# hherlyng/knp-emi-cgx

Hardware: AMD Instinct MI355X
Metric: MDoF/s per implicit timestep (assembly+GMRES) (higher is better)
Workload: dtype f64

## Files before the change

include/knpemi_hip.h:

```cpp
#ifndef KNPEMI_HIP_H
#define KNPEMI_HIP_H

#include <stdint.h>

#ifdef __cplusplus
extern "C" {
#endif

#define KNP_MAX_IONS 3
#define KNP_MAX_AUX 8
#define KNP_DIAG_MAX_CONSTS 64
#define KNP_MAX_PROG_REGS 48
#define KNP_STATE_MAX_INSTR 768
#define KNP_STATE_MAX_CONSTS 128
#define KNP_MAX_AMG_LEVELS 16
#define KNP_FUNCTIONAL_MAX_Q 125

#define KNP_OK 0
#define KNP_E_ARG (-1)
#define KNP_E_HIP (-2)
#define KNP_E_STATE (-3)
#define KNP_E_ALLOC (-4)
#define KNP_E_MESH (-5)

// ... 222 lines not shown
                         double rhs_scale, double* b);
int knp_emi_pc_setup(knp_ctx* ctx, int32_t kind);
int knp_emi_pc_apply(knp_ctx* ctx, const double* r, double* z);
int knp_emi_cg_solve(knp_ctx* ctx, const double* b, double* x, double rtol, double atol, int32_t max_it, int32_t norm_type,
                     int32_t* its, double* rnorm, int32_t* reason);
int knp_emi_update(knp_ctx* ctx, const double* x, double* phi_i, double* phi_e, double* phi_m);

int knp_timer_mark(knp_ctx* ctx, int32_t join_assembly);
int knp_timer_read(knp_ctx* ctx, int32_t capacity, double* seconds , int32_t* n_intervals);
int knp_timer_pending(const knp_ctx* ctx);
int knp_profile_enable(knp_ctx* ctx, int32_t class_mask);
int knp_profile_get(knp_ctx* ctx, int32_t cls, double* ms, int64_t* launches);
int knp_profile_reset(knp_ctx* ctx);
enum { KNP_ST_BNORM = 0 , KNP_ST_ALLREDUCE = 1 ,
       KNP_ST_HALO = 2 , KNP_ST_READBACK = 3 ,
       KNP_ST_FUSED = 4 ,
       KNP_ST_NORM_FALLBACK = 5 ,
       KNP_ST_BLOCKED = 6 ,
       KNP_ST_FUSED_LEVELS = 7 ,
       KNP_ST_FUSED_DOTS = 8 ,
       KNP_ST_SPMV_DOTS = 9 ,
       KNP_ST_FUSED_TAILS = 10 ,
       KNP_ST_KNOD_SKIPS = 11 ,
       KNP_ST_COUNT = 12 };
int knp_get_stats(const knp_ctx* ctx, double* out );
int knp_get_traffic_model(const knp_ctx* ctx, double* out );
enum { KNP_LI_ASM_VARIANT = 0 ,
       KNP_LI_ASM_STAGE = 1 ,
       KNP_LI_ASM_DMAX = 2 ,
       KNP_LI_ASM_GROUP = 3, KNP_LI_SPMV_GROUP = 4, KNP_LI_PC_GROUP = 5 ,
       KNP_LI_MAX_NODE_CELLS = 6 ,
       KNP_LI_MAX_NODE_PAIRS = 7 ,
       KNP_LI_SPMV_UNROLL = 8 ,
       KNP_LI_SPMV_MK = 9 ,
       KNP_LI_COUNT = 10 };
int knp_get_launch_info(const knp_ctx* ctx, int32_t* out , int n);
enum { KNP_AI_A_LANES = 0, KNP_AI_P_LANES = 1, KNP_AI_R_LANES = 2, KNP_AI_S_LANES = 3, KNP_AI_RT_LANES = 4, KNP_AI_U_LANES = 5,
       KNP_AI_BA_LANES = 6, KNP_AI_BR_LANES = 7, KNP_AI_BS_LANES = 8, KNP_AI_BRT_LANES = 9, KNP_AI_BU_LANES = 10,
       KNP_AI_P_N_ACT = 11, KNP_AI_S_N_ACT = 12 ,
       KNP_AI_LFUSED = 13 ,
       KNP_AI_N = 14, KNP_AI_N_COARSE = 15, KNP_AI_FP32 = 16 ,
       KNP_AI_H_FUSED = 17, KNP_AI_H_BLOCKED = 18, KNP_AI_H_CFUSED = 19, KNP_AI_H_L0_FUSED = 20 ,
       KNP_AI_H_NC = 21 ,
       KNP_AI_H_CINV_F32 = 22 ,
       KNP_AI_COUNT = 23 };
int knp_amg_get_level_info(const knp_ctx* ctx, int32_t hier, int32_t level, int32_t* out , int n);

// ... 5 lines not shown
```

knp-emi-cgx_amd/cgx_hip/backend.py:

```python
from __future__ import annotations

import ctypes as C
import os

import numpy as np
import torch

from . import _lib
from ._lib import Fields, FieldsOut, KnpError, MeshDesc
from .parallel import HaloPlan, all_reduce_sum_, guarded


class _CAI:

    def __init__(self, ptr, n):
        self.__cuda_array_interface__ = {"shape": (int(n),), "typestr": "<f8", "data": (int(ptr), False),
                                         "version": 2, "strides": None}


def _f64(a):
    return a.ctypes.data_as(_lib.f64p)


def _i32(a):
# ... 665 lines not shown
    def timer_pending(self):
        return int(self.lib.knp_timer_pending(self.ctx))

    def timer_read(self):
        n = self.timer_pending()
        if n < 2:
            if n:
                out = (C.c_double * 1)()
                k = C.c_int32()
                self.check(self.lib.knp_timer_read(self.ctx, 1, out, C.byref(k)))
            return np.zeros(0)
        out = (C.c_double * n)()
        k = C.c_int32()
        self.check(self.lib.knp_timer_read(self.ctx, n, out, C.byref(k)))
        return np.array(out[:k.value], dtype=np.float64)

    def profile_enable(self, mask=0x1f):
        self.check(self.lib.knp_profile_enable(self.ctx, int(mask)))

    def profile_reset(self):
        self.check(self.lib.knp_profile_reset(self.ctx))

    def stats(self):
        out = (C.c_double * 12)()
        self.check(self.lib.knp_get_stats(self.ctx, out))
        return {"bnorm": out[0], "allreduces": int(out[1]), "halos": int(out[2]), "readbacks": int(out[3]), "fused": int(out[4]),
                "norm_fallbacks": int(out[5]), "blocked": int(out[6]), "fused_levels": int(out[7]),
                "fused_dots": int(out[8]), "spmv_dots": int(out[9]), "fused_tails": int(out[10]), "knod_skips": int(out[11])}

    def nodal_conc(self):
        out = np.empty((self.n_nodes, 4), dtype=np.float64)
        self.check(self.lib.knp_get_nodal_conc(self.ctx, _f64(out)))
        return out

    def traffic_model(self):
        out = (C.c_double * 5)()
        self.check(self.lib.knp_get_traffic_model(self.ctx, out))
        return {"spmv": out[0], "pc": out[1], "assembly_matrix": out[2], "assembly_rhs": out[3], "vector": out[4]}

    def launch_info(self):
        names = ["asm_variant", "asm_stage", "asm_dmax", "asm_group", "spmv_group", "pc_group", "max_node_cells", "max_node_pairs",
                 "spmv_unroll", "spmv_mk"]
        out = (C.c_int32 * len(names))()
        self.check(self.lib.knp_get_launch_info(self.ctx, out, len(names)))
        return dict(zip(names, (int(v) for v in out)))

    AMG_LEVEL_INFO = ["A_lanes", "P_lanes", "R_lanes", "S_lanes", "Rt_lanes", "U_lanes", "bA_lanes", "bR_lanes", "bS_lanes", "bRt_lanes",
                      "bU_lanes", "P_n_act", "S_n_act", "lfused", "n", "n_coarse", "fp32", "fused", "blocked", "cfused", "l0_fused", "nc", "cinv_f32"]

    def amg_level_info(self, hier, level):
        out = (C.c_int32 * len(self.AMG_LEVEL_INFO))()
# ... 13 lines not shown
```

knp-emi-cgx_amd/csrc/knp_internal.hpp:

```cpp
#pragma once
#include <hip/hip_runtime.h>

#include <cstdint>
#include <string>
#include <vector>

#include "knpemi_hip.h"

#define KNP_NPROF 5

struct KnpHostGraph {
    int dim = 0, nv1 = 0;
    int n_v = 0, n_v_owned = 0, n_c = 0, n_c_owned = 0, n_g = 0, n_q = 0;
    int n_nodes = 0, n_nodes_owned = 0;
    std::vector<int32_t> node_i, node_e;
    std::vector<int32_t> node_vertex;
    std::vector<uint8_t> node_side;
    std::vector<int32_t> pair_ptr;
    std::vector<int32_t> pair_col;
    std::vector<int32_t> pair_row;
    std::vector<double> pair_M, pair_K;
    std::vector<int32_t> contrib_ptr;
    std::vector<int32_t> contrib_cell;
    std::vector<double> contrib_k;
// ... 330 lines not shown
    void* comm_user = nullptr;
    KnpP2P* p2p = nullptr;
    int p2p_fine = -1;
    int p2p_red = -1;
    bool hook_allreduce() const { return allreduce && p2p_red < 0; }
    int comm_rc = 0;
    int n_int = 0, n_bnd = 0;
    int32_t *d_nodes_int = nullptr, *d_nodes_bnd = nullptr;
    hipStream_t stream3 = nullptr;
    hipEvent_t ev_x = nullptr, ev_halo = nullptr;
    hipStream_t stream2 = nullptr;
    hipEvent_t ev_fork = nullptr, ev_join = nullptr;
    KnpSidePrep prep;
    bool side_ws = false;
    double *d_t2_s = nullptr, *d_w2_s = nullptr, *d_wb = nullptr, *d_partial_s = nullptr;
    hipStream_t stream_asm = nullptr;
    hipEvent_t ev_fork_asm = nullptr, ev_asm = nullptr;
    bool asm_pending = false;
    double last_bnorm = 0.0;
    int64_t n_allreduce = 0, n_halo = 0, n_readback = 0;
    int64_t n_fused_dots = 0;
    int64_t n_spmv_dots = 0;
    int fused_tail = 1;
    int update_early = 1;
    bool tail_ok = false;
    bool have_tail_target = false;
    knp_fields_out tail_target = {};
    const double* tail_x = nullptr;
    bool fields_current = false, knod_current = false, fields_promise = false;
    bool knod_skipped = false;
    int64_t n_fused_tail = 0;
    int64_t n_knod_skip = 0;
    std::vector<hipEvent_t> tm_events;
    size_t tm_used = 0;
    KnpDiagMap diag_cells, diag_facets;
    KnpDiagMap diag_flux;
    double2* d_flux_rec = nullptr;
    KnpDiagMap diag_phim;
    int32_t* diag_code = nullptr;
    int diag_n_instr = 0, diag_n_regs = 0, diag_n_consts = 0;
    double diag_consts[KNP_DIAG_MAX_CONSTS] = {};
    bool diag_prog = false;
    KnpEmi emi;
    KnpStates states;
    std::vector<KnpSamplePlan> sample_plans;
    std::vector<KnpFunctional> functionals;
// ... 11 lines not shown
```

knp-emi-cgx_amd/csrc/knp_kernels.hip:

```cpp
#include <hip/hip_runtime.h>
#include <hip/hip_ext.h>

#include <algorithm>
#include <cmath>
#include <cstdio>
#include <cstdlib>
#include <cstring>
#include <new>

#include "knp_dispatch.hpp"
#include "knp_internal.hpp"

#define HIPCHK(call)                                                                       \
    do {                                                                                   \
        hipError_t e_ = (call);                                                            \
        if (e_ != hipSuccess) {                                                            \
            ctx->err = std::string(#call) + ": " + hipGetErrorString(e_);                  \
            return KNP_E_HIP;                                                              \
        }                                                                                  \
    } while (0)
#define KCHK(expr)                         \
    do {                                   \
        int rc_ = (expr);                  \
        if (rc_ != KNP_OK) return rc_;     \
// ... 1565 lines not shown
    static const double scale_r = getenv("KNP_LANE_SCALE_R") ? atof(getenv("KNP_LANE_SCALE_R")) : 1.0;
    avg_nnz_per_row *= scale * (role == 1 ? scale_p : role == 2 ? scale_r : 1.0);
    if (avg_nnz_per_row <= 8.0) return 2;
    if (avg_nnz_per_row <= 16.0) return 4;
    if (avg_nnz_per_row <= 32.0) return 8;
    if (avg_nnz_per_row <= 80.0) return 16;
    if (avg_nnz_per_row <= 192.0) return 32;
    return 64;
}

struct GmLayout {
    int m;
    __host__ __device__ int H(int i, int j) const { return i + j * (m + 1); }
    __host__ __device__ int cs() const { return (m + 1) * m; }
    __host__ __device__ int sn() const { return cs() + m; }
    __host__ __device__ int g() const { return sn() + m; }
    __host__ __device__ int y() const { return g() + m + 1; }
    __host__ __device__ int st() const { return y() + m; }
    __host__ __device__ int size() const { return st() + 8; }
};
static constexpr double GM_CANCEL = 1e-8;

__device__ __forceinline__ void givens_body(GmLayout L, int j, int has_ns, double inv_cnt, const double* __restrict__ red, int explicit_slot,
                                            double* __restrict__ gm, double* mirror, volatile int64_t* seq, int64_t seq_val) {
    double* st = gm + L.st();
    double nrm2;
    bool cancel = false;
    if (explicit_slot < 0) {
        const double ww = red[j + 1 + has_ns];
        double s = 0.0;
        for (int i = 0; i <= j; ++i) s += red[i] * red[i];
        if (has_ns) s += red[j + 1] * red[j + 1] * inv_cnt;
        nrm2 = ww - s;
        cancel = !(nrm2 > GM_CANCEL * ww) && ww > 0.0;
    } else {
        nrm2 = red[explicit_slot];
    }
    double flag = 0.0, res = 0.0;
    if (cancel) {
        flag = 1.0;
        nrm2 = 1.0;
    } else {
        double* h = gm + L.H(0, j);
        for (int i = 0; i <= j; ++i) h[i] = red[i];
        h[j + 1] = sqrt(fmax(nrm2, 0.0));
        double* cs = gm + L.cs();
        double* sn = gm + L.sn();
        double* g = gm + L.g();
        for (int i = 0; i < j; ++i) {
            const double t = cs[i] * h[i] + sn[i] * h[i + 1];
            h[i + 1] = -sn[i] * h[i] + cs[i] * h[i + 1];
            h[i] = t;
        }
        const double den = hypot(h[j], h[j + 1]);
        if (!(den > 0.0) || !isfinite(den) || !(nrm2 == nrm2)) {
            flag = 2.0;
            nrm2 = 1.0;
        } else {
            cs[j] = h[j] / den;
            sn[j] = h[j + 1] / den;
            h[j] = den;
            h[j + 1] = 0.0;
            g[j + 1] = -sn[j] * g[j];
            g[j] = cs[j] * g[j];
            res = fabs(g[j + 1]);
            if (!(nrm2 > 0.0)) nrm2 = 1.0;
        }
    }
    st[0] = nrm2; st[1] = flag; st[2] = res;
    if (mirror) { mirror[0] = res; mirror[1] = flag; }
    if (seq) {
        __threadfence_system();
        *seq = seq_val;
    }
}
__global__ void k_givens(GmLayout L, int j, int has_ns, double inv_cnt, const double* __restrict__ red, int explicit_slot,
                         double* __restrict__ gm, double* mirror, volatile int64_t* seq, int64_t seq_val) {
    if (threadIdx.x != 0) return;
    givens_body(L, j, has_ns, inv_cnt, red, explicit_slot, gm, mirror, seq, seq_val);
}

__device__ __forceinline__ void proj_norm_body(double s, double ww, double* __restrict__ red, int slot_out, double inv_count, double cancel, double* mirror,
                                               volatile int64_t* seq, int64_t seq_val) {
    const double nrm2 = ww - s * s * inv_count;
    const bool bad = !(nrm2 > cancel * ww) && ww > 0.0;
    red[slot_out] = bad ? ww : nrm2;
    red[slot_out + 1] = bad ? 1.0 : 0.0;
    if (mirror) { mirror[slot_out] = red[slot_out]; mirror[slot_out + 1] = red[slot_out + 1]; }
    if (seq) {
        __threadfence_system();
        *seq = seq_val;
    }
}
__device__ __forceinline__ void reduce_partial_rows(int nb, int nred, const double* __restrict__ partial, int stride, double* s_red) {
    const int wave = threadIdx.x >> 6, lane = threadIdx.x & 63;
    for (int row = wave; row < nred; row += NT / 64) {
        double a = 0.0;
        for (int c = 0; c < nb; c += 1024) {
            double v[16];
#pragma unroll
            for (int k = 0; k < 16; ++k) {
                const int b = c + lane + 64 * k;
                v[k] = b < nb ? partial[(size_t)row * stride + b] : 0.0;
            }
#pragma unroll
            for (int k = 0; k < 16; ++k) a += v[k];
        }
        a = wave_sum(a);
        if (lane == 0) s_red[row] = a;
    }
    __syncthreads();
}
__global__ void __launch_bounds__(NT)
k_reduce_fin(int mode, int nb, int nred, const double* __restrict__ partial, double* __restrict__ red, int slot0, GmLayout L, int j, int has_ns,
             double inv_cnt, double* __restrict__ gm, int slot_out, double cancel, double* mirror, volatile int64_t* seq, int64_t seq_val,
             int stride = RED_BLOCKS) {
    __shared__ double s_red[RED_SLOTS];
    reduce_partial_rows(nb, nred, partial, stride, s_red);
    if (threadIdx.x < nred) red[slot0 + threadIdx.x] = s_red[threadIdx.x];
// ... 65 lines not shown
            __threadfence_system();
            *seq = seq_val;
        }
    }
}

__global__ void __launch_bounds__(NT) k_dot(int n, const double* __restrict__ a, const double* __restrict__ b,
                                            double* __restrict__ partial) {
    __shared__ double sm[NT / 64];
    double acc = 0.0;
    for (int e = blockIdx.x * NT + threadIdx.x; e < n; e += gridDim.x * NT) acc += a[e] * b[e];
    acc = block_sum(acc, sm);
    if (threadIdx.x == 0) partial[blockIdx.x] = acc;
}

__global__ void __launch_bounds__(NT) k_scale_rsqrt(int n, const double* __restrict__ in, const double* __restrict__ nrm2,
                                                    double* __restrict__ out) {
    const double inv = 1.0 / sqrt(*nrm2);
    for (int e = blockIdx.x * NT + threadIdx.x; e < n; e += gridDim.x * NT) out[e] = in[e] * inv;
}
__global__ void __launch_bounds__(NT) k_scale_rsqrt_proj(int n, const double* __restrict__ in, const double* __restrict__ nrm2,
                                                         const double* __restrict__ phi_sum, double inv_count, double* __restrict__ out,
                                                         double* __restrict__ gm_g = nullptr, int m = 0) {
    if (gm_g && blockIdx.x == 0)
        for (int i = threadIdx.x; i <= m; i += NT) gm_g[i] = (i == 0) ? sqrt(*nrm2) : 0.0;
    const double inv = 1.0 / sqrt(*nrm2);
    const double mean = (*phi_sum) * inv_count;
    for (int e = blockIdx.x * NT + threadIdx.x; e < n; e += gridDim.x * NT) out[e] = ((e & 3) == 3 ? in[e] - mean : in[e]) * inv;
}
__global__ void k_proj_norm(double* __restrict__ red, int slot_s, int slot_out, double inv_count, double cancel, double* mirror,
                            volatile int64_t* seq, int64_t seq_val) {
    if (threadIdx.x != 0) return;
    proj_norm_body(red[slot_s], red[slot_s + 1], red, slot_out, inv_count, cancel, mirror, seq, seq_val);
}
__global__ void __launch_bounds__(NT) k_lincomb(int n, int64_t ldv, int m, const double* __restrict__ V,
                                                const double* __restrict__ y, double* __restrict__ x) {
    for (int e = blockIdx.x * NT + threadIdx.x; e < n; e += gridDim.x * NT) {
        double xe = x[e];
        for (int i = 0; i < m; ++i) xe += y[i] * V[(int64_t)i * ldv + e];
        x[e] = xe;
    }
}

__global__ void k_gm_init(GmLayout L, double* __restrict__ gm, const double* __restrict__ beta2) {
    const int t = threadIdx.x;
    for (int i = t; i <= L.m; i += blockDim.x) gm[L.g() + i] = (i == 0) ? sqrt(*beta2) : 0.0;
}

__global__ void __launch_bounds__(NT)
k_update_scale(int n, int64_t ldv, int m, const double* __restrict__ V, const double* __restrict__ h, const double* __restrict__ w,
               const double* __restrict__ st, double ns_scale, double* __restrict__ out, double ttol) {
    if (ttol > 0.0 && st[1] == 0.0 && st[2] <= ttol) return;
    const double inv = st[1] == 0.0 ? 1.0 / sqrt(st[0]) : 1.0;
    const double mean = ns_scale != 0.0 ? h[m] * ns_scale : 0.0;
    const int n2 = n >> 1;
    for (int e2 = blockIdx.x * NT + threadIdx.x; e2 < n2; e2 += gridDim.x * NT) {
        double2 we = *reinterpret_cast<const double2*>(w + 2 * (size_t)e2);
        if (e2 & 1) we.y -= mean;
        for (int i = 0; i < m; ++i) {
            const double2 v = *reinterpret_cast<const double2*>(V + (int64_t)i * ldv + 2 * (size_t)e2);
            const double hi = h[i];
            we.x -= hi * v.x;
            we.y -= hi * v.y;
        }
        *reinterpret_cast<double2*>(out + 2 * (size_t)e2) = make_double2(we.x * inv, we.y * inv);
    }
}
__global__ void __launch_bounds__(NT) k_scale_inplace_rsqrt(int n, const double* __restrict__ nrm2, double* __restrict__ v) {
    const double inv = 1.0 / sqrt(*nrm2);
    for (int e = blockIdx.x * NT + threadIdx.x; e < n; e += gridDim.x * NT) v[e] *= inv;
}
__global__ void k_gm_solve_y(GmLayout L, int jd, double* __restrict__ gm) {
    if (threadIdx.x != 0) return;
    double* y = gm + L.y();
    const double* g = gm + L.g();
    for (int i = jd - 1; i >= 0; --i) {
        double s = g[i];
        for (int k = i + 1; k < jd; ++k) s -= gm[L.H(i, k)] * y[k];
        y[i] = s / gm[L.H(i, i)];
    }
}

__global__ void __launch_bounds__(NT) k_lincomb_solve(GmLayout L, int jd, double* __restrict__ gm, int n, int64_t ldv,
                                                      const double* __restrict__ V, double* __restrict__ x) {
    __shared__ double sH[8 * 8], sg[8], sy[8];
    if (threadIdx.x < jd * jd) sH[threadIdx.x] = gm[L.H(threadIdx.x % jd, threadIdx.x / jd)];
    if (threadIdx.x < jd) sg[threadIdx.x] = gm[L.g() + threadIdx.x];
    __syncthreads();
// ... 2369 lines not shown

int knp_pc_setup(knp_ctx* ctx, int32_t kind) {
    CHECK_CTX(ctx);
    side_discard(ctx);
    KCHK(join_asm(ctx));
    if (kind != KNP_PC_NONE && kind != KNP_PC_VBJACOBI && kind != KNP_PC_AMG && kind != KNP_PC_AMG_BT && kind != KNP_PC_AMG_LT) { ctx->err = "unknown pc kind"; return KNP_E_ARG; }
    if (kind == KNP_PC_AMG) KCHK(check_hier(ctx, 0));
    if (kind == KNP_PC_AMG_BT || kind == KNP_PC_AMG_LT) {
        KCHK(check_hier(ctx, 0));
        KCHK(check_hier(ctx, 1));
        if (!ctx->d_t2) {
            HIPCHK(hipMalloc((void**)&ctx->d_t2, std::max(ctx->n_dof_local, 1) * sizeof(double)));
            HIPCHK(hipMalloc((void**)&ctx->d_w2, std::max(ctx->n_dof_local, 1) * sizeof(double)));
            HIPCHK(hipMemset(ctx->d_t2, 0, std::max(ctx->n_dof_local, 1) * sizeof(double)));
            HIPCHK(hipMemset(ctx->d_w2, 0, std::max(ctx->n_dof_local, 1) * sizeof(double)));
        }
    }
    ctx->pc_kind = kind;
    ctx->fused_dots = !(getenv("KNP_FUSED_DOTS") && atoi(getenv("KNP_FUSED_DOTS")) == 0);
    ctx->spmv_dots = !(getenv("KNP_SPMV_DOTS") && atoi(getenv("KNP_SPMV_DOTS")) == 0);
    ctx->gmres_ahead = !(getenv("KNP_GMRES_AHEAD") && atoi(getenv("KNP_GMRES_AHEAD")) == 0);
    ctx->fused_tail = !(getenv("KNP_FUSED_TAIL") && atoi(getenv("KNP_FUSED_TAIL")) == 0);
    ctx->update_early = !(getenv("KNP_UPDATE_EARLY") && atoi(getenv("KNP_UPDATE_EARLY")) == 0);
    ctx->fields_current = ctx->knod_current = false;
    for (int h = 0; h < KNP_MAX_HIER; ++h) ctx->hier[h].fused = 0;
    if (kind == KNP_PC_AMG) ctx->hier[0].fused = fused_eligible(ctx, ctx->hier[0]) ? 1 : 0;
    if (kind == KNP_PC_AMG_BT || kind == KNP_PC_AMG_LT) {
        const bool ok = fused_eligible(ctx, ctx->hier[0]) && fused_eligible(ctx, ctx->hier[1]) && ctx->hier[1].native0 == 3 && ctx->hier[0].native0 == 2 &&
                        ctx->hier[1].lv[0].S_n_act > 0 && ctx->hier[1].lv[0].S_act_rows_c && ctx->hier[1].lv[0].R_ci_c;
        ctx->hier[0].fused = ctx->hier[1].fused = ok ? 1 : 0;
        if (!ok && ctx->hier[1].l0_upload) ctx->hier[1].native0 = 0;
    }
    for (int h = 0; h < KNP_MAX_HIER; ++h) {
        KnpAmgHier& H = ctx->hier[h];
        const bool off = getenv("KNP_BLOCKED") && atoi(getenv("KNP_BLOCKED")) == 0;
        bool ok = !off && H.fused && H.node_nf > 0 && (H.native0 == 1 || H.native0 == 2) && (H.native0 == 1) == (H.node_nf == 4);
        for (int l = 0; ok && l < H.levels - 1; ++l) {
            const KnpAmgLevel& L = H.lv[l];
            ok = L.bR.rp && L.bS.rp && (l == 0 || L.bA.rp) && L.bR.n_rows * H.node_nf == L.n_coarse &&
                 L.bS.n_rows * (l == 0 ? 4 : H.node_nf) == L.n;
        }
        H.blocked = ok ? 1 : 0;
        const bool coff = getenv("KNP_COARSE_FUSED") && atoi(getenv("KNP_COARSE_FUSED")) == 0;
        bool cok = !coff && H.fused && H.levels >= 3;
        for (int l = 1; cok && l < H.levels - 1; ++l) {
            const KnpAmgLevel& L = H.lv[l];
// ... 292 lines not shown
}
int knp_timer_pending(const knp_ctx* ctx) { return ctx ? (int)ctx->tm_used : 0; }

int knp_profile_enable(knp_ctx* ctx, int32_t on) {
    CHECK_CTX(ctx);
    KCHK(prof_collect(ctx));
    ctx->prof_on = on;
    return KNP_OK;
}
int knp_profile_get(knp_ctx* ctx, int32_t cls, double* ms, int64_t* launches) {
    CHECK_CTX(ctx);
    if (cls < 0 || cls >= KNP_NPROF || !ms || !launches) return KNP_E_ARG;
    KCHK(prof_collect(ctx));
    *ms = ctx->prof_ms[cls];
    *launches = ctx->prof_n[cls];
    return KNP_OK;
}
int knp_profile_reset(knp_ctx* ctx) {
    CHECK_CTX(ctx);
    KCHK(prof_collect(ctx));
    for (int i = 0; i < KNP_NPROF; ++i) { ctx->prof_ms[i] = 0; ctx->prof_n[i] = 0; }
    ctx->n_allreduce = ctx->n_halo = ctx->n_readback = ctx->n_norm_fallback = 0;
    ctx->n_fused_dots = 0;
    ctx->n_spmv_dots = 0;
    ctx->n_fused_tail = ctx->n_knod_skip = 0;
    return KNP_OK;
}
static double cycle_bytes(const knp_ctx* ctx, const KnpAmgHier& H) {
    if (H.levels < 1) return 0.0;
    const double vs = H.cinv_f || ctx->amg_fp32 ? 4.0 : 8.0;
    double b = 0.0;
    const int nl = H.levels;
    const int nf0 = H.native0 == 1 ? 4 : H.native0 == 2 ? 3 : 1;
    const double n0 = (double)ctx->g.n_nodes_owned;
    auto blocked = [&](const KnpBlockedCsr& M, int nf) { return (double)M.nnz * (nf == 4 ? 20.0 : 16.0) + 4.0 * (M.n_rows + 1); };
    auto scalar = [&](int64_t nnz, int rows) { return (double)nnz * (vs + 4.0) + 4.0 * (rows + 1); };
    if (H.at0_rp) b += scalar(H.lv[0].A_nnz, ctx->g.n_nodes_owned);
    else if (H.native0) b += (double)ctx->n_pairs * (vs * nf0 + 4.0) + 4.0 * (n0 + 1);
    else b += scalar(H.lv[0].A_nnz, H.lv[0].n);
    b += 8.0 * n0 * nf0 * 3.0;
    for (int l = 0; l < nl - 1; ++l) {
        const KnpAmgLevel& L = H.lv[l];
        const double nl_ = (double)(l == 0 ? n0 * nf0 : L.n), nc_ = (double)L.n_coarse;
        const bool mid = l >= 1 && H.cfused;
        if (mid) {
            b += (H.blocked ? blocked(L.bRt, H.node_nf) : scalar(L.Rt_nnz, L.n_coarse)) + 8.0 * (nl_ + nc_);
// ... 25 lines not shown
    out[2] = (double)(ctx->n_tc > 0 ? ctx->n_tc : ctx->n_contrib) * 9.0 + conc + np_ * 32.0 + ngp * (64.0 + 48.0);
    out[3] = no * (8.0 * 4.0 + 9.0) + np_ * (8.0 + 4.0 + 24.0) + (double)g.n_g * g.dim * 7.0 * 8.0 * 2.0;
    out[4] = 8.0 * ctx->n_dof_owned;
    return KNP_OK;
}
int knp_get_stats(const knp_ctx* ctx, double* out) {
    if (!ctx || !out) return KNP_E_ARG;
    for (int i = 0; i < KNP_ST_COUNT; ++i) out[i] = 0.0;
    out[KNP_ST_BNORM] = ctx->last_bnorm;
    out[KNP_ST_ALLREDUCE] = (double)ctx->n_allreduce;
    out[KNP_ST_HALO] = (double)ctx->n_halo;
    out[KNP_ST_READBACK] = (double)ctx->n_readback;
    out[KNP_ST_FUSED] = (double)(ctx->hier[0].fused + 2 * ctx->hier[1].fused + 4 * ctx->hier[0].l0_fused + 8 * ctx->hier[1].l0_fused);
    out[KNP_ST_NORM_FALLBACK] = (double)ctx->n_norm_fallback;
    out[KNP_ST_BLOCKED] = (double)(ctx->hier[0].blocked + 2 * ctx->hier[1].blocked);
    int nlf = 0;
    for (int h = 0; h < KNP_MAX_HIER; ++h)
        for (int l = 1; l < ctx->hier[h].levels; ++l) nlf += ctx->hier[h].lv[l].lfused;
    out[KNP_ST_FUSED_LEVELS] = (double)nlf;
    out[KNP_ST_FUSED_DOTS] = (double)ctx->n_fused_dots;
    out[KNP_ST_SPMV_DOTS] = (double)ctx->n_spmv_dots;
    out[KNP_ST_FUSED_TAILS] = (double)ctx->n_fused_tail;
    out[KNP_ST_KNOD_SKIPS] = (double)ctx->n_knod_skip;
    return KNP_OK;
}
int knp_get_launch_info(const knp_ctx* ctx, int32_t* out, int n) {
    if (!ctx || !out || n <= 0) return KNP_E_ARG;
    const KnpHostGraph& g = ctx->g;
    int32_t v[KNP_LI_COUNT];
    v[KNP_LI_ASM_VARIANT] = ctx->asm_stage > 0 ? (ctx->d_tc_meta ? 2 : 1) : 0;
    v[KNP_LI_ASM_STAGE] = ctx->asm_stage;
    v[KNP_LI_ASM_DMAX] = ctx->asm_dmax;
    v[KNP_LI_ASM_GROUP] = ctx->asm_group;
    v[KNP_LI_SPMV_GROUP] = ctx->spmv_group;
    v[KNP_LI_PC_GROUP] = ctx->pc_group;
    v[KNP_LI_MAX_NODE_CELLS] = g.max_node_cells;
    int dmax = 0;
    if ((int)g.pair_ptr.size() > g.n_nodes_owned)
        for (int node = 0; node < g.n_nodes_owned; ++node) dmax = std::max(dmax, g.pair_ptr[node + 1] - g.pair_ptr[node]);
    v[KNP_LI_MAX_NODE_PAIRS] = dmax;
    static const int unroll = getenv("KNP_SPMV_UNROLL") ? atoi(getenv("KNP_SPMV_UNROLL")) : 2;
    static const bool mf_off = getenv("KNP_SPMV_MF") && atoi(getenv("KNP_SPMV_MF")) == 0;
    v[KNP_LI_SPMV_UNROLL] = unroll >= 2 ? 2 : 1;
    v[KNP_LI_SPMV_MK] = (!mf_off && ctx->n_bc == 0 && ctx->d_pair_MK != nullptr) ? 1 : 0;
    for (int i = 0; i < n && i < KNP_LI_COUNT; ++i) out[i] = v[i];
    return KNP_OK;
// ... 48 lines not shown
```

knp-emi-cgx_amd/csrc/knp_krylov.inc:

```

static constexpr int GM_RES = 100, GM_EXPL = 57, GM_MAX_RESTART = GM_EXPL - 2;
static constexpr int FB_SLOT = 124;
static_assert(GM_RES + 2 <= RED_SLOTS && DEFL_SLOT0 + DEFL_MAX <= GM_RES, "reduction slot layout");
static constexpr double GM_DTOL = 1e5;

static void side_discard(knp_ctx* ctx) {
    switch (ctx->prep.kind) {
        case KnpSidePrep::NONE:
        case KnpSidePrep::LEFT_DEFERRED: break;
        default: (void)hipEventSynchronize(ctx->ev_join);
    }
    ctx->prep.kind = KnpSidePrep::NONE;
}
static int ensure_side_stream(knp_ctx* ctx) {
    if (ctx->stream2) return KNP_OK;
    HIPCHK(hipStreamCreateWithFlags(&ctx->stream2, hipStreamNonBlocking));
    HIPCHK(hipEventCreateWithFlags(&ctx->ev_fork, hipEventDisableTiming));
    HIPCHK(hipEventCreateWithFlags(&ctx->ev_join, hipEventDisableTiming));
    return KNP_OK;
}

static bool exchanges_all_native(const knp_ctx* ctx) {
    if (!ctx->p2p || ctx->p2p_fine < 0 || ctx->p2p_red < 0 || ctx->defl_m > 0) return false;
    const int nh = ctx->pc_kind == KNP_PC_AMG ? 1 : (ctx->pc_kind == KNP_PC_AMG_BT || ctx->pc_kind == KNP_PC_AMG_LT) ? 2 : 0;
    for (int h = 0; h < nh; ++h)
        for (int l = 0; l < ctx->hier[h].levels; ++l) {
            const KnpAmgLevel& L = ctx->hier[h].lv[l];
            if (L.dist && L.p2p_halo < 0) return false;
            if (L.repl_n > 0 && L.p2p_repl < 0) return false;
        }
    return true;
}

static bool fin_ok(const knp_ctx* ctx) {
    static const bool off = getenv("KNP_FIN") && atoi(getenv("KNP_FIN")) == 0;
    return !off && !ctx->allreduce && ctx->p2p_red < 0;
}
static bool fused_norm_possible(const knp_ctx* ctx, int64_t cnt) {
    static const bool off = getenv("KNP_NO_FUSED_NORM") != nullptr;
    return ctx->ns_on && cnt > 0 && !off && ctx->defl_m == 0;
}
static int pc_apply_norm(knp_ctx* ctx, const double* r, double* z, int64_t cnt, bool* fused, bool side = false) {
    if (side) {
        *fused = true;
        DotReq dq{0, true, (int64_t)ctx->n_dof_local, ctx->d_V, ctx->d_partial_s};
        KCHK(pc_apply_proj(ctx, r, z, 0, (ctx->fused_dots && fin_ok(ctx)) ? &dq : nullptr));
        ProfScope ps(ctx, 1);
        const int nb = dq.done ? dq.nb : ctx->n_red_blocks;
        if (!dq.done)
            hipLaunchKernelGGL((k_multi_dot<8, true, true>), dim3(nb), dim3(NT), 0, ctx->stream, ctx->n_dof_owned, (int64_t)ctx->n_dof_local, 0, 0,
                               ctx->d_V, z, ctx->d_partial_s);
        ++ctx->n_allreduce;
        hipLaunchKernelGGL(k_reduce_fin, dim3(1), dim3(NT), 0, ctx->stream, 2, nb, 2, ctx->d_partial_s, ctx->d_red, SIDE_SLOT + 2, GmLayout{1}, 0, 0,
                           1.0 / (double)cnt, (double*)nullptr, SIDE_SLOT, GM_CANCEL, ctx->mirror(), (volatile int64_t*)nullptr, (int64_t)0,
                           dq.done ? RED_WIDE : RED_BLOCKS);
        HIPCHK(hipGetLastError());
        return KNP_OK;
    }
    if (!fused_norm_possible(ctx, cnt)) {
        *fused = false;
        KCHK(pc_apply_proj(ctx, r, z, cnt));
        return dot_to_slot(ctx, z, z, 60);
    }
    *fused = true;
    DotReq dq{0, true, (int64_t)ctx->n_dof_local, ctx->d_V, ctx->d_partial};
    KCHK(pc_apply_proj(ctx, r, z, 0, (ctx->fused_dots && fin_ok(ctx)) ? &dq : nullptr));
    ProfScope ps(ctx, 1);
    const int nb = dq.done ? dq.nb : ctx->n_red_blocks;
    if (!dq.done)
        hipLaunchKernelGGL((k_multi_dot<8, true, true>), dim3(nb), dim3(NT), 0, ctx->stream, ctx->n_dof_owned, (int64_t)ctx->n_dof_local, 0, 0,
                           ctx->d_V, z, ctx->d_partial);
    if (fin_ok(ctx)) {
        ++ctx->n_allreduce;
        hipLaunchKernelGGL(k_reduce_fin, dim3(1), dim3(NT), 0, ctx->stream, 2, nb, 2, ctx->d_partial, ctx->d_red, 62, GmLayout{1}, 0, 0, 1.0 / (double)cnt,
                           (double*)nullptr, 60, GM_CANCEL, ctx->mirror(), ctx->mirror() ? ctx->h_seq_dev : nullptr, ++ctx->seq_counter,
                           dq.done ? RED_WIDE : RED_BLOCKS);
        HIPCHK(hipGetLastError());
        return KNP_OK;
    }
    hipLaunchKernelGGL(k_reduce_partials, dim3(2), dim3(NT), 0, ctx->stream, nb, ctx->d_partial, ctx->d_red, 62, (double*)nullptr);
    KCHK(allreduce_slots(ctx, 62, 2));
    hipLaunchKernelGGL(k_proj_norm, dim3(1), dim3(64), 0, ctx->stream, ctx->d_red, 62, 60, 1.0 / (double)cnt, GM_CANCEL, ctx->mirror(),
                       ctx->mirror() ? ctx->h_seq_dev : nullptr, ++ctx->seq_counter);
    HIPCHK(hipGetLastError());
    return KNP_OK;
}
static int pc_norm_read(knp_ctx* ctx, double* z, int64_t cnt, bool* fused) {
    KCHK(read_slots(ctx, 60, *fused ? 2 : 1, ctx->seq_counter));
    if (*fused && ctx->h_red[61] != 0.0) {
        ++ctx->n_norm_fallback;
        const int no = ctx->g.n_nodes_owned;
        hipLaunchKernelGGL(k_phi_sub, dim3(nblocks(no)), dim3(NT), 0, ctx->stream, no, ctx->d_red + 62, 1.0 / (double)cnt, z);
        *fused = false;
        KCHK(dot_to_slot(ctx, z, z, 60));
// ... 166 lines not shown
    return KNP_OK;
}

static int arnoldi_step_enqueue(const KrylovSolve& K, int j, const double* w, double* vn, int first_nb, int first_stride, double early = 0.0) {
    knp_ctx* ctx = K.ctx;
    hipStream_t st = ctx->stream;
    const GmLayout GL = K.GL;
    double* gm = K.gm;
    const int n = K.n, nb = K.nb, nsi = K.ns ? 1 : 0;
    const int64_t ldv = K.ldv;
    ProfScope ps(ctx, 1);
    const bool done = first_nb > 0;
    const int nbr = done ? first_nb : nb;
    const int pst = done ? first_stride : RED_BLOCKS;
    for (int i0 = 0; i0 <= j && !done; i0 += 8) {
        if (i0 == 0 && K.ns)
            hipLaunchKernelGGL((k_multi_dot<8, true, true>), dim3(nb), dim3(NT), 0, st, n, ldv, i0, j + 1, ctx->d_V, w, ctx->d_partial);
        else if (i0 == 0)
            hipLaunchKernelGGL((k_multi_dot<8, false, true>), dim3(nb), dim3(NT), 0, st, n, ldv, i0, j + 1, ctx->d_V, w, ctx->d_partial);
        else
            hipLaunchKernelGGL((k_multi_dot<8, false, false>), dim3(nb), dim3(NT), 0, st, n, ldv, i0, j + 1, ctx->d_V, w, ctx->d_partial);
    }
    const int nred = j + 2 + nsi;
    if (fin_ok(ctx)) {
        ++ctx->n_allreduce;
        hipLaunchKernelGGL(k_reduce_fin, dim3(1), dim3(NT), 0, st, 1, nbr, nred, ctx->d_partial, ctx->d_red, 0, GL, j, nsi, K.inv_cnt, gm,
                           0, 0.0, ctx->mirror() ? ctx->h_red_dev + GM_RES : nullptr, ctx->mirror() ? ctx->h_seq_dev : nullptr, ++ctx->seq_counter,
                           pst);
    } else {
        hipLaunchKernelGGL(k_reduce_partials, dim3(nred), dim3(NT), 0, st, nbr, ctx->d_partial, ctx->d_red, 0, (double*)nullptr);
        KCHK(allreduce_slots(ctx, 0, nred));
        hipLaunchKernelGGL(k_givens, dim3(1), dim3(64), 0, st, GL, j, nsi, K.inv_cnt, ctx->d_red, -1, gm,
                           ctx->mirror() ? ctx->h_red_dev + GM_RES : nullptr, ctx->mirror() ? ctx->h_seq_dev : nullptr, ++ctx->seq_counter);
    }
    hipLaunchKernelGGL(k_update_scale, dim3(nb), dim3(NT), 0, st, n, ldv, j + 1, ctx->d_V, ctx->d_red, w, gm + GL.st(), K.inv_cnt, vn, early);
    HIPCHK(hipGetLastError());
    return KNP_OK;
}
static int arnoldi_step_read(const KrylovSolve& K, int j, double* vn, double* res, int* flag, bool have = false) {
    knp_ctx* ctx = K.ctx;
    hipStream_t st = ctx->stream;
    const GmLayout GL = K.GL;
    double* gm = K.gm;
    const int n = K.n, nb = K.nb, nsi = K.ns ? 1 : 0;
    if (!have) KCHK(gm_read_state(K, res, flag));
    if (*flag == 1) {
// ... 75 lines not shown
            ++ctx->n_norm_fallback;
            KCHK(pc_apply_proj(ctx, b, ctx->d_w, cnt));
            KCHK(dot_to_slot(ctx, ctx->d_w, ctx->d_w, 60));
            KCHK(read_slots(ctx, 60, 1, ctx->seq_counter));
        }
    } else {
        side_discard(ctx);
        bool fused_norm = false;
        KCHK(pc_apply_norm(ctx, b, ctx->d_w, cnt, &fused_norm));
        KCHK(pc_norm_read(ctx, ctx->d_w, cnt, &fused_norm));
    }
    double bnorm = lazy_bnorm ? 0.0 : std::sqrt(ctx->h_red[60]);
    ctx->last_bnorm = bnorm;
    if (!lazy_bnorm && !std::isfinite(bnorm)) { *its = 0; *rnorm = bnorm; *reason = KNP_DIVERGED_NANORINF; return KNP_OK; }
    K.ttol = std::max(rtol * bnorm, atol);
    K.atol = atol;
    int it = 0;
    double res = 0.0, res0 = -1.0;
    *reason = 0;
    const bool ns = ctx->ns_on && cnt > 0;
    K.ns = ns;
    K.inv_cnt = ns ? 1.0 / (double)cnt : 0.0;
    auto enqueue_v0 = [&](bool fused_norm) {
        if (fused_norm) {
            hipLaunchKernelGGL(k_scale_rsqrt_proj, dim3(K.vec_blocks), dim3(NT), 0, st, n, ctx->d_w, ctx->d_red + 60, ctx->d_red + 62,
                               1.0 / (double)cnt, ctx->d_V, gm + GL.g(), m);
        } else {
            hipLaunchKernelGGL(k_scale_rsqrt, dim3(K.vec_blocks), dim3(NT), 0, st, n, ctx->d_w, ctx->d_red + 60, ctx->d_V);
            hipLaunchKernelGGL(k_gm_init, dim3(1), dim3(64), 0, st, GL, gm, ctx->d_red + 60);
        }
    };
    auto enqueue_iteration = [&](int j, double early) -> int {
        double* vj = ctx->d_V + (size_t)j * ldv;
        double* vn = ctx->d_V + (size_t)(j + 1) * ldv;
        KCHK(spmv_A(ctx, vj, nullptr, ctx->d_t, false));
        DotReq dq{j + 1, ns, ldv, ctx->d_V, ctx->d_partial};
        KCHK(pc_apply_proj(ctx, ctx->d_t, ctx->d_w, ns ? 0 : cnt, (ctx->fused_dots && fin_ok(ctx) && j + 1 <= BU_MAX_M) ? &dq : nullptr));
        return arnoldi_step_enqueue(K, j, ctx->d_w, vn, dq.done ? dq.nb : 0, RED_WIDE, early);
    };
    const bool ahead_ok = ctx->gmres_ahead && ctx->mirror() && ctx->h_seq && ctx->h_seq_dev && !ctx->halo && !ctx->allreduce && !ctx->p2p &&
                          !ctx->level_comm && ctx->defl_m == 0 && ctx->n_bc == 0 && max_it > 0 && (ctx->prof_on & ~1) == 0;
    const bool tail_ok = ctx->fused_tail && ctx->tail_ok && ctx->have_tail_target && !ctx->halo && !ctx->allreduce && !ctx->level_comm && !ctx->p2p &&
                         ctx->defl_m == 0 && ctx->n_bc == 0 && (ctx->prof_on & ~1) == 0;
    while (true) {
        KCHK(spmv_A(ctx, x, b, ctx->d_t, true));
        bool fused_norm = false;
        KCHK(pc_apply_norm(ctx, ctx->d_t, ctx->d_w, cnt, &fused_norm));
        if (lazy_bnorm && ctx->prep.kind == KnpSidePrep::LEFT_DEFERRED) {
            ctx->prep.kind = KnpSidePrep::LEFT_CONCURRENT;
            HIPCHK(hipStreamWaitEvent(ctx->stream2, ctx->ev_fork, 0));
            ctx->stream = ctx->stream2;
            bool fn = false;
            swap_side_ws(ctx);
            const int rcs = pc_apply_norm(ctx, b, ctx->d_wb, cnt, &fn, true);
            swap_side_ws(ctx);
            ctx->stream = st;
            KCHK(rcs);
            HIPCHK(hipEventRecord(ctx->ev_join, ctx->stream2));
        }
        bool ahead = ahead_ok && fused_norm;
        double res_a = 0.0;
        int flag_a = 0;
        auto redo_residual = [&]() -> int {
            if (ahead) KCHK(spmv_A(ctx, x, b, ctx->d_t, true));
            ahead = false;
            KCHK(pc_apply_norm(ctx, ctx->d_t, ctx->d_w, cnt, &fused_norm));
            return pc_norm_read(ctx, ctx->d_w, cnt, &fused_norm);
        };
        if (ahead) {
            enqueue_v0(true);
// ... 150 lines not shown
```

Measured before the change: 2246.

## Fuse final reduction, Givens update and Arnoldi vector update into one multi-block kernel

Adds k_fin_update, which reduces the dot-product partials redundantly in every block, has each block run the Givens rotation locally (block 0 publishes it), and then performs the orthogonalization update and normalization of the new Krylov vector. This replaces the separate single-block k_reduce_fin followed by k_update_scale. A matching k_fin_v0 fuses the deferred norm reduction with scaling of the initial vector v0. The aim is to remove a kernel launch and a serialized single-block reduction per Arnoldi step, at the cost of every block redundantly reading the partials and a more intricate state handoff through gm slots.

```diff
diff --git a/include/knpemi_hip.h b/include/knpemi_hip.h
--- a/include/knpemi_hip.h
+++ b/include/knpemi_hip.h
@@ -268,7 +268,9 @@
        KNP_ST_SPMV_DOTS = 9 ,
        KNP_ST_FUSED_TAILS = 10 ,
        KNP_ST_KNOD_SKIPS = 11 ,
-       KNP_ST_COUNT = 12 };
+       KNP_ST_FIN_UPDATE = 12 ,
+       KNP_ST_FIN_V0 = 13 ,
+       KNP_ST_COUNT = 14 };
 int knp_get_stats(const knp_ctx* ctx, double* out );
 int knp_get_traffic_model(const knp_ctx* ctx, double* out );
 enum { KNP_LI_ASM_VARIANT = 0 ,
diff --git a/knp-emi-cgx_amd/cgx_hip/backend.py b/knp-emi-cgx_amd/cgx_hip/backend.py
--- a/knp-emi-cgx_amd/cgx_hip/backend.py
+++ b/knp-emi-cgx_amd/cgx_hip/backend.py
@@ -711,11 +711,12 @@
         self.check(self.lib.knp_profile_reset(self.ctx))
 
     def stats(self):
-        out = (C.c_double * 12)()
+        out = (C.c_double * 14)()
         self.check(self.lib.knp_get_stats(self.ctx, out))
         return {"bnorm": out[0], "allreduces": int(out[1]), "halos": int(out[2]), "readbacks": int(out[3]), "fused": int(out[4]),
                 "norm_fallbacks": int(out[5]), "blocked": int(out[6]), "fused_levels": int(out[7]),
-                "fused_dots": int(out[8]), "spmv_dots": int(out[9]), "fused_tails": int(out[10]), "knod_skips": int(out[11])}
+                "fused_dots": int(out[8]), "spmv_dots": int(out[9]), "fused_tails": int(out[10]), "knod_skips": int(out[11]),
+                "fin_updates": int(out[12]), "fin_v0s": int(out[13])}
 
     def nodal_conc(self):
         out = np.empty((self.n_nodes, 4), dtype=np.float64)
diff --git a/knp-emi-cgx_amd/csrc/knp_internal.hpp b/knp-emi-cgx_amd/csrc/knp_internal.hpp
--- a/knp-emi-cgx_amd/csrc/knp_internal.hpp
+++ b/knp-emi-cgx_amd/csrc/knp_internal.hpp
@@ -376,6 +376,11 @@
     int64_t n_fused_dots = 0;
     int64_t n_spmv_dots = 0;
     int fused_tail = 1;
+    int fin_update = 1;
+    int fin_update_blocks = 256;
+    int64_t n_fin_update = 0;
+    int64_t n_fin_v0 = 0;
+    struct { int nb = 0, stride = 0; int64_t seq = 0; } fin_pend;
     int update_early = 1;
     bool tail_ok = false;
     bool have_tail_target = false;
diff --git a/knp-emi-cgx_amd/csrc/knp_kernels.hip b/knp-emi-cgx_amd/csrc/knp_kernels.hip
--- a/knp-emi-cgx_amd/csrc/knp_kernels.hip
+++ b/knp-emi-cgx_amd/csrc/knp_kernels.hip
@@ -1611,7 +1611,8 @@
 static constexpr double GM_CANCEL = 1e-8;
 
 __device__ __forceinline__ void givens_body(GmLayout L, int j, int has_ns, double inv_cnt, const double* __restrict__ red, int explicit_slot,
-                                            double* __restrict__ gm, double* mirror, volatile int64_t* seq, int64_t seq_val) {
+                                            double* __restrict__ gm, double* mirror, volatile int64_t* seq, int64_t seq_val, double* hc = nullptr,
+                                            bool pub = true, double* out3 = nullptr) {
     double* st = gm + L.st();
     double nrm2;
     bool cancel = false;
@@ -1630,7 +1631,7 @@
         flag = 1.0;
         nrm2 = 1.0;
     } else {
-        double* h = gm + L.H(0, j);
+        double* h = hc ? hc : gm + L.H(0, j);
         for (int i = 0; i <= j; ++i) h[i] = red[i];
         h[j + 1] = sqrt(fmax(nrm2, 0.0));
         double* cs = gm + L.cs();
@@ -1646,16 +1647,24 @@
             flag = 2.0;
             nrm2 = 1.0;
         } else {
-            cs[j] = h[j] / den;
-            sn[j] = h[j + 1] / den;
-            h[j] = den;
-            h[j + 1] = 0.0;
-            g[j + 1] = -sn[j] * g[j];
-            g[j] = cs[j] * g[j];
-            res = fabs(g[j + 1]);
+            const double gj = pub ? g[j] : st[4 + (j & 1)];
+            const double csj = h[j] / den, snj = h[j + 1] / den;
+            const double gn = -snj * gj;
+            if (pub) {
+                cs[j] = csj;
+                sn[j] = snj;
+                h[j] = den;
+                h[j + 1] = 0.0;
+                g[j + 1] = gn;
+                g[j] = csj * gj;
+                st[4 + ((j + 1) & 1)] = gn;
+            }
+            res = fabs(gn);
             if (!(nrm2 > 0.0)) nrm2 = 1.0;
         }
     }
+    if (out3) { out3[0] = nrm2; out3[1] = flag; out3[2] = res; }
+    if (!pub) return;
     st[0] = nrm2; st[1] = flag; st[2] = res;
     if (mirror) { mirror[0] = res; mirror[1] = flag; }
     if (seq) {
@@ -1669,11 +1678,16 @@
     givens_body(L, j, has_ns, inv_cnt, red, explicit_slot, gm, mirror, seq, seq_val);
 }
 
+__device__ __forceinline__ double proj_norm_value(double s, double ww, double inv_count, double cancel, bool* flagged) {
+    const double nrm2 = ww - s * s * inv_count;
+    const bool bad = !(nrm2 > cancel * ww) && ww > 0.0;
+    *flagged = bad;
+    return bad ? ww : nrm2;
+}
 __device__ __forceinline__ void proj_norm_body(double s, double ww, double* __restrict__ red, int slot_out, double inv_count, double cancel, double* mirror,
                                                volatile int64_t* seq, int64_t seq_val) {
-    const double nrm2 = ww - s * s * inv_count;
-    const bool bad = !(nrm2 > cancel * ww) && ww > 0.0;
-    red[slot_out] = bad ? ww : nrm2;
+    bool bad;
+    red[slot_out] = proj_norm_value(s, ww, inv_count, cancel, &bad);
     red[slot_out + 1] = bad ? 1.0 : 0.0;
     if (mirror) { mirror[slot_out] = red[slot_out]; mirror[slot_out + 1] = red[slot_out + 1]; }
     if (seq) {
@@ -1681,9 +1695,10 @@
         *seq = seq_val;
     }
 }
+template <int BT = NT>
 __device__ __forceinline__ void reduce_partial_rows(int nb, int nred, const double* __restrict__ partial, int stride, double* s_red) {
     const int wave = threadIdx.x >> 6, lane = threadIdx.x & 63;
-    for (int row = wave; row < nred; row += NT / 64) {
+    for (int row = wave; row < nred; row += BT / 64) {
         double a = 0.0;
         for (int c = 0; c < nb; c += 1024) {
             double v[16];
@@ -1795,8 +1810,10 @@
 __global__ void __launch_bounds__(NT) k_scale_rsqrt_proj(int n, const double* __restrict__ in, const double* __restrict__ nrm2,
                                                          const double* __restrict__ phi_sum, double inv_count, double* __restrict__ out,
                                                          double* __restrict__ gm_g = nullptr, int m = 0) {
-    if (gm_g && blockIdx.x == 0)
+    if (gm_g && blockIdx.x == 0) {
         for (int i = threadIdx.x; i <= m; i += NT) gm_g[i] = (i == 0) ? sqrt(*nrm2) : 0.0;
+        if (threadIdx.x == 0) gm_g[2 * m + 1 + 4] = sqrt(*nrm2);
+    }
     const double inv = 1.0 / sqrt(*nrm2);
     const double mean = (*phi_sum) * inv_count;
     for (int e = blockIdx.x * NT + threadIdx.x; e < n; e += gridDim.x * NT) out[e] = ((e & 3) == 3 ? in[e] - mean : in[e]) * inv;
@@ -1818,6 +1835,7 @@
 __global__ void k_gm_init(GmLayout L, double* __restrict__ gm, const double* __restrict__ beta2) {
     const int t = threadIdx.x;
     for (int i = t; i <= L.m; i += blockDim.x) gm[L.g() + i] = (i == 0) ? sqrt(*beta2) : 0.0;
+    if (t == 0) gm[L.st() + 4] = sqrt(*beta2);
 }
 
 __global__ void __launch_bounds__(NT)
@@ -1837,6 +1855,67 @@
             we.y -= hi * v.y;
         }
         *reinterpret_cast<double2*>(out + 2 * (size_t)e2) = make_double2(we.x * inv, we.y * inv);
+    }
+}
+static constexpr int FU_NT = 1024, FU_MAX_BLOCKS = 256;
+__global__ void __launch_bounds__(FU_NT)
+k_fin_update(int nb, int nred, const double* __restrict__ partial, int stride, double* __restrict__ red, GmLayout L, int j, int has_ns,
+             double inv_cnt, double* gm, double* mirror, volatile int64_t* seq, int64_t seq_val, int n, int64_t ldv,
+             const double* __restrict__ V, const double* __restrict__ w, double* __restrict__ out, double ttol) {
+    __shared__ double s_red[RED_SLOTS], s_h[RED_SLOTS], s_st[3];
+    reduce_partial_rows<FU_NT>(nb, nred, partial, stride, s_red);
+    const bool own = blockIdx.x == 0;
+    if (own && threadIdx.x < nred) red[threadIdx.x] = s_red[threadIdx.x];
+    if (threadIdx.x == 0) givens_body(L, j, has_ns, inv_cnt, s_red, -1, gm, mirror, seq, seq_val, own ? nullptr : s_h, own, s_st);
+    __syncthreads();
+    if (ttol > 0.0 && s_st[1] == 0.0 && s_st[2] <= ttol) return;
+    const double inv = s_st[1] == 0.0 ? 1.0 / sqrt(s_st[0]) : 1.0;
+    const int m = j + 1;
+    const double mean = inv_cnt != 0.0 ? s_red[m] * inv_cnt : 0.0;
+    const int n2 = n >> 1, step = gridDim.x * FU_NT;
+    for (int ea = blockIdx.x * FU_NT + threadIdx.x; ea < n2; ea += 2 * step) {
+        const int eb = ea + step;
+        const bool hb = eb < n2;
+        double2 wa = *reinterpret_cast<const double2*>(w + 2 * (size_t)ea);
+        double2 wb = hb ? *reinterpret_cast<const double2*>(w + 2 * (size_t)eb) : make_double2(0.0, 0.0);
+        if (ea & 1) wa.y -= mean;
+        if (eb & 1) wb.y -= mean;
+        for (int i = 0; i < m; ++i) {
+            const double2 va = *reinterpret_cast<const double2*>(V + (int64_t)i * ldv + 2 * (size_t)ea);
+            const double2 vb = hb ? *reinterpret_cast<const double2*>(V + (int64_t)i * ldv + 2 * (size_t)eb) : make_double2(0.0, 0.0);
+            const double hi = s_red[i];
+            wa.x -= hi * va.x;
+            wa.y -= hi * va.y;
+            wb.x -= hi * vb.x;
+            wb.y -= hi * vb.y;
+        }
+        *reinterpret_cast<double2*>(out + 2 * (size_t)ea) = make_double2(wa.x * inv, wa.y * inv);
+        if (hb) *reinterpret_cast<double2*>(out + 2 * (size_t)eb) = make_double2(wb.x * inv, wb.y * inv);
+    }
+}
+__global__ void __launch_bounds__(FU_NT)
+k_fin_v0(int nb, const double* __restrict__ partial, int stride, double* __restrict__ red, int slot0, int slot_out, double inv_count, double cancel,
+         double* mirror, volatile int64_t* seq, int64_t seq_val, int n, const double* __restrict__ in, double* __restrict__ out,
+         double* __restrict__ gm_g, int m) {
+    __shared__ double s_red[RED_SLOTS];
+    reduce_partial_rows<FU_NT>(nb, 2, partial, stride, s_red);
+    bool bad;
+    const double s = s_red[0], nrm2 = proj_norm_value(s, s_red[1], inv_count, cancel, &bad);
+    if (blockIdx.x == 0) {
+        if (threadIdx.x < 2) red[slot0 + threadIdx.x] = s_red[threadIdx.x];
+        for (int i = threadIdx.x; i <= m; i += FU_NT) gm_g[i] = (i == 0) ? sqrt(nrm2) : 0.0;
+        if (threadIdx.x == 0) {
+            gm_g[2 * m + 1 + 4] = sqrt(nrm2);
+            proj_norm_body(s, s_red[1], red, slot_out, inv_count, cancel, mirror, seq, seq_val);
+        }
+    }
+    const double inv = 1.0 / sqrt(nrm2);
+    const double mean = s * inv_count;
+    const int n2 = n >> 1;
+    for (int e2 = blockIdx.x * FU_NT + threadIdx.x; e2 < n2; e2 += gridDim.x * FU_NT) {
+        double2 v = *reinterpret_cast<const double2*>(in + 2 * (size_t)e2);
+        if (e2 & 1) v.y -= mean;
+        *reinterpret_cast<double2*>(out + 2 * (size_t)e2) = make_double2(v.x * inv, v.y * inv);
     }
 }
 __global__ void __launch_bounds__(NT) k_scale_inplace_rsqrt(int n, const double* __restrict__ nrm2, double* __restrict__ v) {
@@ -4252,6 +4331,8 @@
     ctx->gmres_ahead = !(getenv("KNP_GMRES_AHEAD") && atoi(getenv("KNP_GMRES_AHEAD")) == 0);
     ctx->fused_tail = !(getenv("KNP_FUSED_TAIL") && atoi(getenv("KNP_FUSED_TAIL")) == 0);
     ctx->update_early = !(getenv("KNP_UPDATE_EARLY") && atoi(getenv("KNP_UPDATE_EARLY")) == 0);
+    ctx->fin_update = !(getenv("KNP_FIN_UPDATE") && atoi(getenv("KNP_FIN_UPDATE")) == 0);
+    ctx->fin_update_blocks = getenv("KNP_FIN_UPDATE_BLOCKS") ? std::min(std::max(atoi(getenv("KNP_FIN_UPDATE_BLOCKS")), 1), FU_MAX_BLOCKS) : FU_MAX_BLOCKS;
     ctx->fields_current = ctx->knod_current = false;
     for (int h = 0; h < KNP_MAX_HIER; ++h) ctx->hier[h].fused = 0;
     if (kind == KNP_PC_AMG) ctx->hier[0].fused = fused_eligible(ctx, ctx->hier[0]) ? 1 : 0;
@@ -4590,6 +4671,7 @@
     for (int i = 0; i < KNP_NPROF; ++i) { ctx->prof_ms[i] = 0; ctx->prof_n[i] = 0; }
     ctx->n_allreduce = ctx->n_halo = ctx->n_readback = ctx->n_norm_fallback = 0;
     ctx->n_fused_dots = 0;
+    ctx->n_fin_update = ctx->n_fin_v0 = 0;
     ctx->n_spmv_dots = 0;
     ctx->n_fused_tail = ctx->n_knod_skip = 0;
     return KNP_OK;
@@ -4661,6 +4743,8 @@
     out[KNP_ST_SPMV_DOTS] = (double)ctx->n_spmv_dots;
     out[KNP_ST_FUSED_TAILS] = (double)ctx->n_fused_tail;
     out[KNP_ST_KNOD_SKIPS] = (double)ctx->n_knod_skip;
+    out[KNP_ST_FIN_UPDATE] = (double)ctx->n_fin_update;
+    out[KNP_ST_FIN_V0] = (double)ctx->n_fin_v0;
     return KNP_OK;
 }
 int knp_get_launch_info(const knp_ctx* ctx, int32_t* out, int n) {
diff --git a/knp-emi-cgx_amd/csrc/knp_krylov.inc b/knp-emi-cgx_amd/csrc/knp_krylov.inc
--- a/knp-emi-cgx_amd/csrc/knp_krylov.inc
+++ b/knp-emi-cgx_amd/csrc/knp_krylov.inc
@@ -40,7 +40,7 @@
     static const bool off = getenv("KNP_NO_FUSED_NORM") != nullptr;
     return ctx->ns_on && cnt > 0 && !off && ctx->defl_m == 0;
 }
-static int pc_apply_norm(knp_ctx* ctx, const double* r, double* z, int64_t cnt, bool* fused, bool side = false) {
+static int pc_apply_norm(knp_ctx* ctx, const double* r, double* z, int64_t cnt, bool* fused, bool side = false, bool defer = false) {
     if (side) {
         *fused = true;
         DotReq dq{0, true, (int64_t)ctx->n_dof_local, ctx->d_V, ctx->d_partial_s};
@@ -57,6 +57,7 @@
         HIPCHK(hipGetLastError());
         return KNP_OK;
     }
+    ctx->fin_pend.nb = 0;
     if (!fused_norm_possible(ctx, cnt)) {
         *fused = false;
         KCHK(pc_apply_proj(ctx, r, z, cnt));
@@ -70,6 +71,14 @@
     if (!dq.done)
         hipLaunchKernelGGL((k_multi_dot<8, true, true>), dim3(nb), dim3(NT), 0, ctx->stream, ctx->n_dof_owned, (int64_t)ctx->n_dof_local, 0, 0,
                            ctx->d_V, z, ctx->d_partial);
+    if (fin_ok(ctx) && defer) {
+        ++ctx->n_allreduce;
+        ctx->fin_pend.nb = nb;
+        ctx->fin_pend.stride = dq.done ? RED_WIDE : RED_BLOCKS;
+        ctx->fin_pend.seq = ++ctx->seq_counter;
+        HIPCHK(hipGetLastError());
+        return KNP_OK;
+    }
     if (fin_ok(ctx)) {
         ++ctx->n_allreduce;
         hipLaunchKernelGGL(k_reduce_fin, dim3(1), dim3(NT), 0, ctx->stream, 2, nb, 2, ctx->d_partial, ctx->d_red, 62, GmLayout{1}, 0, 0, 1.0 / (double)cnt,
@@ -282,6 +291,16 @@
             hipLaunchKernelGGL((k_multi_dot<8, false, false>), dim3(nb), dim3(NT), 0, st, n, ldv, i0, j + 1, ctx->d_V, w, ctx->d_partial);
     }
     const int nred = j + 2 + nsi;
+    if (fin_ok(ctx) && ctx->fin_update) {
+        ++ctx->n_allreduce;
+        ++ctx->n_fin_update;
+        const int fb = std::max(1, std::min(ctx->fin_update_blocks, ((n >> 1) + 2 * FU_NT - 1) / (2 * FU_NT)));
+        hipLaunchKernelGGL(k_fin_update, dim3(fb), dim3(FU_NT), 0, st, nbr, nred, ctx->d_partial, pst, ctx->d_red, GL, j, nsi, K.inv_cnt, gm,
+                           ctx->mirror() ? ctx->h_red_dev + GM_RES : nullptr, ctx->mirror() ? ctx->h_seq_dev : nullptr, ++ctx->seq_counter,
+                           n, ldv, ctx->d_V, w, vn, early);
+        HIPCHK(hipGetLastError());
+        return KNP_OK;
+    }
     if (fin_ok(ctx)) {
         ++ctx->n_allreduce;
         hipLaunchKernelGGL(k_reduce_fin, dim3(1), dim3(NT), 0, st, 1, nbr, nred, ctx->d_partial, ctx->d_red, 0, GL, j, nsi, K.inv_cnt, gm,
@@ -403,7 +422,14 @@
     K.ns = ns;
     K.inv_cnt = ns ? 1.0 / (double)cnt : 0.0;
     auto enqueue_v0 = [&](bool fused_norm) {
-        if (fused_norm) {
+        if (ctx->fin_pend.nb > 0) {
+            const int fb = std::max(1, std::min(ctx->fin_update_blocks, ((n >> 1) + 2 * FU_NT - 1) / (2 * FU_NT)));
+            hipLaunchKernelGGL(k_fin_v0, dim3(fb), dim3(FU_NT), 0, st, ctx->fin_pend.nb, ctx->d_partial, ctx->fin_pend.stride, ctx->d_red, 62, 60,
+                               1.0 / (double)cnt, GM_CANCEL, ctx->mirror(), ctx->mirror() ? ctx->h_seq_dev : nullptr, ctx->fin_pend.seq, n, ctx->d_w,
+                               ctx->d_V, gm + GL.g(), m);
+            ctx->fin_pend.nb = 0;
+            ++ctx->n_fin_v0;
+        } else if (fused_norm) {
             hipLaunchKernelGGL(k_scale_rsqrt_proj, dim3(K.vec_blocks), dim3(NT), 0, st, n, ctx->d_w, ctx->d_red + 60, ctx->d_red + 62,
                                1.0 / (double)cnt, ctx->d_V, gm + GL.g(), m);
         } else {
@@ -426,7 +452,7 @@
     while (true) {
         KCHK(spmv_A(ctx, x, b, ctx->d_t, true));
         bool fused_norm = false;
-        KCHK(pc_apply_norm(ctx, ctx->d_t, ctx->d_w, cnt, &fused_norm));
+        KCHK(pc_apply_norm(ctx, ctx->d_t, ctx->d_w, cnt, &fused_norm, false, ahead_ok && ctx->fin_update && fused_norm_possible(ctx, cnt)));
         if (lazy_bnorm && ctx->prep.kind == KnpSidePrep::LEFT_DEFERRED) {
             ctx->prep.kind = KnpSidePrep::LEFT_CONCURRENT;
             HIPCHK(hipStreamWaitEvent(ctx->stream2, ctx->ev_fork, 0));
```

After: 2263 (median of 6 runs). No clear change (+0.7%).
